# dannyfa/VAE-GAM

Hardware: AMD Instinct MI355X
Metric: fMRI volumes/sec/train-step (41x49x35) (higher is better)
Workload: dtype f32; 1 GPU; configs[2] full VAE-GAM: B=64/GPU C=8, 41x49x35, 2 subj x 98 vol synthetic checker, fwd+bwd+Adam, hipGraph replay; global_batch=64, covariates=8, parallelism=dp1

## Files before the change

vae-gam_amd/csrc/vg_conv_mm.hip:

```cpp
#include "vg_common.h"
#include <stdlib.h>
#include <stdint.h>
#include "../../include/vaegam.h"

#ifdef VG_STAMP
__device__ unsigned long long vg_stamp_out[1024 * 16 * 8];
#define VG_STAMP_T(t) do { __builtin_amdgcn_sched_barrier(0); asm volatile("s_memtime %0\n\ts_waitcnt lgkmcnt(0)" : "=s"(t) :: "memory"); __builtin_amdgcn_sched_barrier(0); } while (0)
#define VG_STAMP_ADD(i) do { unsigned long long t_; VG_STAMP_T(t_); st_sum[i] += t_ - st_last; st_last = t_; } while (0)
#else
#define VG_STAMP_ADD(i) do {} while (0)
#endif

namespace {

constexpr int MM_MAXQ = 4;
constexpr int MM_ZPAD = 64;

struct MmParams {
    vg_mm_desc d;
    int bps, nsplit;
    int ksbase[MM_MAXQ], a_off[MM_MAXQ];
    int kstot, aimg_floats;
    int a_res;
    int CHP, buf_floats;
// ... 150 lines not shown
        const char* mn = reinterpret_cast<const char*>(mask_src + (size_t)n * CO * ovol);
        const int cq = d.od0[q] * OHW + d.oh0[q] * d.OW + d.ow0[q];
#pragma unroll
        for (int i = 0; i < TPC; ++i) {
            if (i >= nact || !((vbits >> (q * TPC + i)) & 1u)) continue;
            const unsigned off = 4u * (unsigned)(ob[i] + cq);
#pragma unroll
            for (int r = 0; r < 4; ++r) {
                float v = acc[i].v[r] + bias_l[r];
                if constexpr (MASKED) {
                    if constexpr (NQ == 1) v = (mreg[i][r] > 0.f) ? v : 0.f;
                    else v = (*reinterpret_cast<const float*>(mn + (size_t)r * ovol * 4 + off) > 0.f) ? v : 0.f;
                }
#if defined(VG_ABLATE_STORE) && VG_ABLATE_STORE == 1
                if (v == 1.2345e-30f) *reinterpret_cast<float*>(yn + (size_t)r * ovol * 4 + off) = v;
#elif defined(VG_ABLATE_STORE) && VG_ABLATE_STORE == 2
                *reinterpret_cast<float*>(yn + (size_t)r * ovol * 4 + (((off >> 8) << 8) + 4u * lane)) = v;
#elif defined(VG_ABLATE_STORE) && VG_ABLATE_STORE == 4
                if (r == 0 || v == 1.2345e-30f) *reinterpret_cast<float*>(yn + (size_t)r * ovol * 4 + off) = v;
#elif defined(VG_ABLATE_STORE) && VG_ABLATE_STORE == 5
                *reinterpret_cast<float*>(yn + off) = v;
#elif defined(VG_ABLATE_STORE) && VG_ABLATE_STORE == 3
                __builtin_nontemporal_store(v, reinterpret_cast<float*>(yn + (size_t)r * ovol * 4 + off));
#else
                *reinterpret_cast<float*>(yn + (size_t)r * ovol * 4 + off) = v;
#endif
                if (stats_part) {
                    const float h = stats_relu ? vg_max(v, 0.f) : v;
                    st_s[r] += h; st_q[r] = fmaf(h, h, st_q[r]);
                }
            }
        }
    };
    auto flush_stats = [&](int n) __attribute__((always_inline)) {
        const int g = n / stats_pg;
        const size_t chunks = (size_t)stats_pg * p.bps * MM_W;
        const size_t chunkid = ((size_t)(n % stats_pg) * p.bps + b) * MM_W + wave;
#pragma unroll
        for (int r = 0; r < 4; ++r) {
            float sa = st_s[r], sb = st_q[r];
#pragma unroll
            for (int off = 8; off > 0; off >>= 1) { sa += __shfl_xor(sa, off); sb += __shfl_xor(sb, off); }
            if (CO == 8) { sa += __shfl_xor(sa, 32); sb += __shfl_xor(sb, 32); }
            if (jl == 0 && (CO == 16 || kk < 2)) {
                double* dst = stats_part + (((size_t)g * CO + co_l + r) * chunks + chunkid) * 2;
                dst[0] = (double)sa; dst[1] = (double)sb;
            }
            st_s[r] = 0.f; st_q[r] = 0.f;
        }
    };

    const int nsp = d.cc * nspan_c;
    const int parts = (nsp >= MM_W) ? 1 : (MM_W + nsp - 1) / nsp;
    const int head = dst0 & 3;
    const int n4 = (head + span_fl + 3) >> 2;
    const int n4p = (n4 + parts - 1) / parts;
    auto stage = [&](int u) __attribute__((always_inline)) {
        const int n = split + (u / nchunks) * p.nsplit, c0 = (u % nchunks) * d.cc;
        const int cc = min(d.cc, CI - c0);
        float* buf = In + (DB ? (u & 1) : 0) * p.buf_floats;
        const float* src0 = x + ((size_t)n * CI + c0) * vol + (size_t)pl_lo * IHW + (size_t)r_lo * d.IW;
        for (int it = wave; it < cc * nspan_c * parts; it += MM_W) {
            const int sp = it / parts, part = it - sp * parts;
            const int c = sp / nspan_c, pl = sp - c * nspan_c;
            const int g0 = part * n4p, g1 = min(g0 + n4p, n4);
            const int f0 = max(g0 * 4 - head, 0), f1 = min(g1 * 4 - head, span_fl);
            if (f1 > f0) vg_dma_block(src0 + (size_t)c * vol + (size_t)pl * IHW + f0, buf + c * p.CHP + MM_ZPAD + dst0 + pl * LPH + f0, f1 - f0, 0, 1, lane);
        }
    };
    auto prologue = [&](int u) __attribute__((always_inline)) {
        const int n = split + (u / nchunks) * p.nsplit, c0 = (u % nchunks) * d.cc;
        const int cc = min(d.cc, CI - c0);
        float* buf = In + (DB ? (u & 1) : 0) * p.buf_floats;
        const int g_aff = (in_scale != nullptr) ? n / d.per_group : 0;
        for (int it = wave; it < cc * nspan_c * parts; it += MM_W) {
            const int sp = it / parts, part = it - sp * parts;
            const int c = sp / nspan_c, pl = sp - c * nspan_c;
            float sc = 1.f, sh = 0.f;
            if (in_scale != nullptr) { sc = in_scale[g_aff * CI + c0 + c]; sh = in_shift[g_aff * CI + c0 + c]; }
            float* sp0 = buf + c * p.CHP + MM_ZPAD + dst0 + pl * LPH - head;
            const int g0 = part * n4p, g1 = min((part + 1) * n4p, n4);
#ifdef VG_EMU
            for (int g = g0 + lane; g < g1; g += VG_WAVE) {
                float* t = sp0 + g * 4;
#pragma unroll
                for (int e = 0; e < 4; ++e) t[e] = fmaf(vg_max(t[e], lo), sc, sh);
            }
#else
            for (int g = g0 + lane; g < g1; g += VG_WAVE) {
                const unsigned a = (unsigned)(uintptr_t)(sp0 + g * 4);
                vg_hw_f32x4 t;
                asm volatile("ds_read_b128 %0, %1\n\ts_waitcnt lgkmcnt(0)" : "=v"(t) : "v"(a) : "memory");
#pragma unroll
                for (int e = 0; e < 4; ++e) t[e] = fmaf(vg_max(t[e], lo), sc, sh);
                asm volatile("ds_write_b128 %0, %1" :: "v"(a), "v"(t) : "memory");
            }
#endif
        }
#ifndef VG_EMU
        asm volatile("s_waitcnt lgkmcnt(0)" ::: "memory");
#endif
    };
    __syncthreads();
#ifdef VG_STAMP
    unsigned long long st_sum[8] = {0, 0, 0, 0, 0, 0, 0, 0}, st_last;
    VG_STAMP_T(st_last);
#endif
    if (units > 0) stage(0);
    int g_run = -1, n_run = 0;
    int pend = 0;
    for (int u = 0; u < units; ++u) {
        const int n = split + (u / nchunks) * p.nsplit, chunk = u % nchunks, c0 = chunk * d.cc;
        const int cc = min(d.cc, CI - c0);
        float* cur = In + (DB ? (u & 1) : 0) * p.buf_floats;
        VG_STAMP_ADD(7);
        if (DB) vg_dma_wait_wave();
        else vg_wait_vm(pend);
        VG_STAMP_ADD(0);
        if (p.has_pro) prologue(u);
        VG_STAMP_ADD(1);
        __syncthreads();
        VG_STAMP_ADD(2);
        if (DB && u + 1 < units) stage(u + 1);
        if constexpr (NQ == 1 && MASKED) { if (chunk == nchunks - 1) load_mask(n); }
        VG_STAMP_ADD(3);
        auto class_work = [&](auto qc, auto ntc) __attribute__((always_inline)) {
            constexpr int q = decltype(qc)::value;
            constexpr int NT = decltype(ntc)::value;
            for (int c = 0; c < cc; ++c) {
                const float* curc = cur + c * p.CHP;
                if constexpr (STATIC_K) {
                    constexpr int KSQ = q == 0 ? K0 : q == 1 ? K1 : q == 2 ? K2 : K3;
                    constexpr int SG0 = q == 0 ? 0 : q == 1 ? K0 : q == 2 ? K0 + K1 : K0 + K1 + K2;
                    const float* Aq = Al + p.a_off[q] + (c0 + c) * KSQ * 64 + lane;
#ifdef VG_EMU
#pragma unroll
                    for (int s = 0; s < KSQ; ++s) {
                        const float aw = Aq[s * 64];
#pragma unroll
                        for (int i = 0; i < NT; ++i) vg_mfma16(aw, curc[pt[i][SG0 + s]], acc[i]);
                    }
#else
// ... 7 lines not shown
                        if (s + 1 < KSQ) {
                            asm volatile("ds_read_b32 %0, %1 offset:%2" : "=v"(a2[(s + 1) & 1]) : "v"(ab), "n"((s + 1) * 256));
#pragma unroll
                            for (int i = 0; i < NT; ++i)
                                asm volatile("ds_read_b32 %0, %1" : "=v"(b2[(s + 1) & 1][i]) : "v"(cb + 4u * (unsigned)pt[i][SG0 + s + 1]));
                            asm volatile("s_waitcnt lgkmcnt(%0)" :: "n"(NT + 1) : "memory");
                        } else {
                            asm volatile("s_waitcnt lgkmcnt(0)" ::: "memory");
                        }
                        __builtin_amdgcn_sched_barrier(0);
#pragma unroll
                        for (int i = 0; i < NT; ++i) vg_mfma16(a2[s & 1], b2[s & 1][i], acc[i]);
                        __builtin_amdgcn_sched_barrier(0);
                    }
#endif
                } else {
                    const int ksq = d.ks[q];
                    const float* Aq = Al + p.a_off[q] + (c0 + c) * ksq * 64 + lane;
                    const int* Tq = Tl + p.ksbase[q] * 64 + lane;
                    for (int s = 0; s < ksq; ++s) {
                        const float aw = Aq[s * 64];
                        const int off = Tq[s * 64] + MM_ZPAD;
                        const unsigned bit = 1u << s;
                        float bv[NT];
#pragma unroll
                        for (int i = 0; i < NT; ++i) bv[i] = curc[(vm[q][i] & bit) ? posBase[i] + off : 0];
#pragma unroll
                        for (int i = 0; i < NT; ++i) vg_mfma16(aw, bv[i], acc[i]);
                    }
                }
            }
        };
        const int g_now = stats_part ? n / stats_pg : 0;
        if (stats_part && chunk == 0 && g_run >= 0 && g_now != g_run) flush_stats(n_run);
        if constexpr (NQ == 1) {
            if (chunk == 0) zero_acc();
            if (nact > 0) mm_dispatch<TPC>(nact, [&](auto ntc) __attribute__((always_inline)) { class_work(mm_int<0>{}, ntc); });
            VG_STAMP_ADD(4);
            pend = 0;
            if constexpr (!DB) {
                if (u + 1 < units) { __syncthreads(); VG_STAMP_ADD(2); stage(u + 1); VG_STAMP_ADD(3); }
                if (chunk == nchunks - 1) pend = nst[0];
            }
            if (chunk == nchunks - 1) store_class(n, 0);
            VG_STAMP_ADD(5);
        } else {
            mm_static_for<NQ>([&](auto qc) __attribute__((always_inline)) {
                constexpr int q = decltype(qc)::value;
                zero_acc();
                VG_STAMP_ADD(5);
                if (nact > 0) mm_dispatch<TPC>(nact, [&](auto ntc) __attribute__((always_inline)) { class_work(qc, ntc); });
                VG_STAMP_ADD(4);
                if constexpr (!DB && q == NQ - 1) {
                    if (u + 1 < units) { __syncthreads(); VG_STAMP_ADD(2); stage(u + 1); VG_STAMP_ADD(3); }
                    pend = nst[q];
                }
                store_class(n, q);
            });
            VG_STAMP_ADD(5);
        }
        g_run = g_now; n_run = n;
    }
    if (stats_part && g_run >= 0) flush_stats(n_run);
    VG_STAMP_ADD(6);
#ifdef VG_STAMP
    if (lane == 0 && blockIdx.x < 1024)
        for (int i = 0; i < 8; ++i) vg_stamp_out[(blockIdx.x * 16 + wave) * 8 + i] = st_sum[i];
#endif
}

}

#ifdef VG_STAMP
extern "C" int vg_stamp_read(unsigned long long* dst, int n) {
    return (int)hipMemcpyFromSymbol(dst, HIP_SYMBOL(vg_stamp_out), sizeof(unsigned long long) * n, 0, hipMemcpyDeviceToHost);
}
#endif

static int mm_plan_params(const vg_mm_desc* d, MmParams* p, size_t* shmem, const char* who) {
    if (!d || d->N <= 0 || d->CI <= 0 || (d->CO != 8 && d->CO != 16) || d->nq < 1 || d->nq > MM_MAXQ || d->PD <= 0 || d->PDT <= 0 ||
        d->PH <= 0 || d->PW <= 0 || d->slack < 0 || d->PH > 1023 || d->PW > 1023 || d->PD > 1023 || d->cc <= 0 || d->LD <= 0 || d->tpc <= 0) {
        vg_set_error("%s: bad descriptor", who); return VG_ERR_ARG;
    }
    p->d = *d;
    int ns = 256 / p->bps; if (ns < 1) ns = 1; if (ns > d->N) ns = d->N;
    p->nsplit = ns;
    int row = 0, af = 0;
    for (int q = 0; q < d->nq; ++q) {
        if (d->ks[q] <= 0 || d->ks[q] > 32) { vg_set_error("%s: k-steps per channel must be 1..32 (class %d: %d)", who, q, d->ks[q]); return VG_ERR_ARG; }
        p->ksbase[q] = row; p->a_off[q] = af;
        row += d->ks[q]; af += d->CI * d->ks[q] * 64;
    }
    p->kstot = row; p->aimg_floats = af;
    if (d->nq > 1 && d->cc < d->CI) { vg_set_error("%s: multi-class plans need all input channels in one chunk", who); return VG_ERR_ARG; }
    const int IHW = d->IH * d->IW;
    const int W = d->waves;
// ... 92 lines not shown
```

vae-gam_amd/csrc/vg_gp.hip:

```cpp
#include "vg_common.h"
#include "../../include/vaegam.h"

namespace {

constexpr int GP_T = 256;
constexpr int GP_TB = 1024;
constexpr int GP_LDS_MAXB = 16;
constexpr int GP_NB = 16;
constexpr int GP_NBP = GP_NB + 1;
constexpr int TAB_W = 10;

struct GpLayout {
    long long Lc, A, kinv, Ls, M, N1, N2, N3, N4, T1, T2, T3, G, x, e, bm, v1, v2, v3, sc, total;
};

__host__ __device__ inline GpLayout gp_layout(long long B, long long n) {
    GpLayout w; long long o = 0;
    w.Lc = o; o += B * B;
    w.A = o; o += B * n;
    w.kinv = o; o += n * n;
    w.Ls = o; o += n * n;
    w.M = o; o += n * n;
    w.N1 = o; o += n * n; w.N2 = o; o += n * n; w.N3 = o; o += n * n; w.N4 = o; o += n * n;
    w.T1 = o; o += B * n; w.T2 = o; o += B * n; w.T3 = o; o += B * n;
// ... 231 lines not shown
            const int b = t / n, k = t % n;
            double s = 0.0;
            for (int j = 0; j < n; ++j) s += T1[b * n + j] * kinv[j * n + k];
            A[t] = s;
        }
        for (int t = tid; t < n * n; t += nt) {
            const int p = t / n, q = t % n;
            M[t] = (double)qS[t] - kvar * (kern1(fabs((double)(p - q)) * step, isl) + (p == q ? a.jitter_ku : 0.0));
        }
        __syncthreads();
        for (int b = tid; b < B; b += nt) {
            double s = 0.0;
            for (int k = 0; k < n; ++k) s += A[b * n + k] * (double)qm[k];
            if (o_fb) o_fb[(size_t)c * B + b] = s;
            bm[b] += s;
        }
        for (int t = tid; t < B * n; t += nt) {
            const int b = t / n, k = t % n;
            double s = 0.0;
            for (int j = 0; j < n; ++j) s += A[b * n + j] * M[j * n + k];
            T2[t] = s;
        }
        for (int t = tid; t < n * n; t += nt) Ls[t] = (double)qS[t];
        __syncthreads();
        chol_inplace(Ls, n);
        double part = 0.0;
        for (int t = tid; t < n * n; t += nt) {
            const int p = t / n, q = t % n;
            if (q <= p) part += Ls[t] * Ls[t] / a.prior_var;
            if (q == p) part += -2.0 * log(Ls[t]) + (double)qm[p] * (double)qm[p] / a.prior_var;
        }
        const double tot = block_sum(part, red);
        kl += 0.5 * (n * log(a.prior_var) + tot - n);
    }
    return kl;
}

template <int T>
__global__ void __launch_bounds__(T)
gain_fwd_k(GainArgs a, float* __restrict__ task_var, double* __restrict__ kl_part,
           double* __restrict__ o_bm, double* __restrict__ o_bc, double* __restrict__ o_fb, double* __restrict__ o_sg) {
    VG_DYN_SMEM(double, lds);
    double* red = lds;
    const int c = blockIdx.x, tid = threadIdx.x, nt = blockDim.x;
    const int B = a.B, n = a.n;
    const GpLayout w = gp_layout(B, n);
    double* W = a.ws + (size_t)c * w.total;
    const bool in_lds = B <= GP_LDS_MAXB;
    double* Cm = in_lds ? lds + T : W + w.Lc;
    const long long* tb = a.tab + (size_t)c * TAB_W;
    const bool is_gp = tb[0] != 0, is_hrf = tb[1] != 0;
    double* x = W + w.x; double* e = W + w.e; double* bm = W + w.bm;
    const double sa = (double)a.P[tb[3]], std_ = exp((double)a.P[tb[4]]);
    double kvar, ls, step;
    const double kl = gain_prelude(a, c, W, w, red, o_fb, kvar, ls, step);
    {
        const double* A = W + w.A; const double* T2 = W + w.T2;
        const double isl = 1.0 / sqrt(2.0) / ls;
        const double s2 = std_ * std_;
        for (long long t = tid; t < (long long)B * B; t += nt) {
            const int i = (int)(t / B), j = (int)(t % B);
            double v = (i == j) ? s2 * x[i] * x[i] : 0.0;
            if (is_gp) {
                double sg = kvar * kern1(x[j] - x[i], isl);
                for (int k = 0; k < n; ++k) sg += T2[i * n + k] * A[j * n + k];
                if (o_sg) o_sg[((size_t)c * B + i) * B + j] = sg;
                v += sg;
            }
            if (o_bc) o_bc[((size_t)c * B + i) * B + j] = v;
            Cm[t] = v + (i == j ? a.jitter_b : 0.0);
        }
        if (o_bm) for (int b = tid; b < B; b += nt) o_bm[(size_t)c * B + b] = bm[b];
    }
    __syncthreads();
    if (in_lds) chol_inplace(Cm, B);
    else chol_blocked(Cm, B, lds + T);
    if (in_lds) {
        double* Lc = W + w.Lc;
        for (long long t = tid; t < (long long)B * B; t += nt) Lc[t] = Cm[t];
    }
    double* tv = W + w.v1;
    if (in_lds) {
        for (int b = tid; b < B; b += nt) {
            double s = bm[b];
            for (int j = 0; j <= b; ++j) s += Cm[(long long)b * B + j] * e[j];
            tv[b] = s;
        }
    } else {
        const int lane = tid % VG_WAVE, wv = tid / VG_WAVE, nwv = nt / VG_WAVE;
        for (int b = wv; b < B; b += nwv) {
            double s = 0.0;
            for (int j = lane; j <= b; j += VG_WAVE) s += Cm[(long long)b * B + j] * e[j];
            for (int off = VG_WAVE / 2; off > 0; off >>= 1) s += __shfl_down(s, off);
            if (lane == 0) tv[b] = bm[b] + s;
        }
    }
    __syncthreads();
    for (int b = tid; b < B; b += nt) {
        double s = tv[b];
        if (is_hrf) {
// ... 326 lines not shown
#pragma unroll
    for (int p = 0; p < 4; ++p)
#pragma unroll
        for (int q = 0; q < 4; ++q) {
            const int i = min(i0 + ty * 4 + p, B - 1), j = min(j0 + tx * 4 + q, B - 1);
            acc[p][q] = is_gp ? kvar * kern1(x[j] - x[i], isl) : 0.0;
        }
    if (is_gp) {
        const double* A = W + w.A; const double* T2 = W + w.T2;
        double* Ts = lds; double* As = lds + GT * GTP;
        for (int k0 = 0; k0 < n; k0 += GT) {
            const int kc = min(GT, n - k0);
            __syncthreads();
            for (int t = tid; t < GT * GT; t += GP_TT) {
                const int r = t / GT, k = t % GT;
                const bool ok = k < kc;
                Ts[k * GTP + r] = (ok && i0 + r < B) ? T2[(long long)(i0 + r) * n + k0 + k] : 0.0;
                As[k * GTP + r] = (ok && j0 + r < B) ? A[(long long)(j0 + r) * n + k0 + k] : 0.0;
            }
            __syncthreads();
            mm4x4(Ts, As, kc, acc);
        }
    }
#pragma unroll
    for (int p = 0; p < 4; ++p)
#pragma unroll
        for (int q = 0; q < 4; ++q) {
            const int i = i0 + ty * 4 + p, j = j0 + tx * 4 + q;
            if (i >= B || j >= B) continue;
            double v = (i == j) ? s2 * x[i] * x[i] : 0.0;
            if (is_gp) {
                if (o_sg) o_sg[((size_t)c * B + i) * B + j] = acc[p][q];
                v += acc[p][q];
            }
            if (o_bc) o_bc[((size_t)c * B + i) * B + j] = v;
            Lc[(long long)i * B + j] = (j > i) ? 0.0 : v + (i == j ? a.jitter_b : 0.0);
        }
}

__global__ void __launch_bounds__(GP_TT)
gain_potrf_diag_k(GainArgs a, int p) {
    VG_DYN_SMEM(double, D);
    const int B = a.B, c = blockIdx.x, tid = threadIdx.x;
    const GpLayout w = gp_layout(B, a.n);
    double* Lc = a.ws + (size_t)c * w.total + w.Lc;
    const int k0 = p * GT, nb = min(GT, B - k0);
    for (int t = tid; t < nb * nb; t += GP_TT) { const int i = t / nb, j = t % nb; D[i * GTP + j] = Lc[(long long)(k0 + i) * B + k0 + j]; }
    for (int j = 0; j < nb; ++j) {
        __syncthreads();
        const double d = sqrt(D[j * GTP + j]);
        __syncthreads();
        for (int i = j + tid; i < nb; i += GP_TT) D[i * GTP + j] = (i == j) ? d : D[i * GTP + j] / d;
        __syncthreads();
        for (int t = tid; t < (nb - j - 1) * (nb - j - 1); t += GP_TT) {
            const int i = j + 1 + t / (nb - j - 1), k = j + 1 + t % (nb - j - 1);
            if (k <= i) D[i * GTP + k] -= D[i * GTP + j] * D[k * GTP + j];
        }
    }
    __syncthreads();
    for (int t = tid; t < nb * nb; t += GP_TT) { const int i = t / nb, j = t % nb; if (j <= i) Lc[(long long)(k0 + i) * B + k0 + j] = D[i * GTP + j]; }
}

__global__ void __launch_bounds__(GP_TT)
gain_potrf_panel_k(GainArgs a, int p) {
    VG_DYN_SMEM(double, lds);
    const int B = a.B, T = gt_tiles(B), tid = threadIdx.x;
// ... 453 lines not shown
```

vae-gam_amd/ops.py:

```python
import ctypes
from dataclasses import dataclass
from typing import Optional, Tuple

import torch

from . import _lib
from ._lib import ConvDesc, WgradDesc

BN_EPS = 1e-5

PROFILE = None
_LABEL = ['']


class label:
    def __init__(self, name):
        self.name = name

    def __enter__(self):
        self.prev = _LABEL[0]; _LABEL[0] = self.name

    def __exit__(self, *a):
        _LABEL[0] = self.prev

# ... 328 lines not shown
    _call(p, 'vg_bn_param_grad', _p(src), G, C, _p(dg), _p(db), 0)
    return dg, db


_GROUPED_OK = {}


def _grouped_wgrad_ok(p_shape, per_group):
    key = (tuple(p_shape), int(per_group))
    if key not in _GROUPED_OK:
        N, C, ID, IH, IW = key[0]
        d = WgradDesc(N, C, 1, ID, IH, IW, ID + 2, IH + 2, IW + 2, 3, 3, 3, 1, 0, 0, 0, 0, 0, int(per_group))
        _GROUPED_OK[key] = _lib.get_lib().dll.vg_wgrad3d_grouped_ws_bytes(ctypes.byref(d)) >= 0
    return _GROUPED_OK[key]


def bn_backward_tconv1(dy, weight, p, gamma, mean, rstd, relu, per_group, sync=None, beta=None, producer_bias_grad=None, dw_out=None):
    lib = _lib.get_lib()
    N, C = p.shape[0], p.shape[1]
    ID, IH, IW = p.shape[2:]
    assert tuple(dy.shape) == (N, 1, ID + 2, IH + 2, IW + 2) and tuple(weight.shape) == (C, 1, 3, 3, 3)
    _chk(dy); _chk(p)
    w = _chk(weight.detach().contiguous())
    G = N // per_group
    P = ID * IH * IW
    ws = torch.empty(lib.size('vg_bn_tconv1_ws_bytes', N, C, ID, per_group) // 8, dtype=torch.float64, device=p.device)
    sums = torch.empty((G * C, 2), dtype=torch.float64, device=p.device)
    if dw_out is not None:
        assert dw_out.shape == weight.shape and dw_out.is_contiguous() and dw_out.dtype == torch.float32 and beta is not None
        d = WgradDesc(N, C, 1, ID, IH, IW, ID + 2, IH + 2, IW + 2, 3, 3, 3, 1, 0, 0, 0, 0, int(relu), int(per_group))
        nbytes = lib.size('vg_wgrad3d_grouped_ws_bytes', ctypes.byref(d))
        wws = torch.empty(nbytes // 4, dtype=torch.float32, device=p.device)
        q = torch.empty((G, C + 1, 27), dtype=torch.float32, device=p.device)
        nshift = -(mean * rstd)
        _call(p, 'vg_wgrad3d_grouped', ctypes.byref(d), _p(dy), _p(p), _p(rstd), _p(nshift), _p(wws), _p(q))
        _call(p, 'vg_bn_tconv1_sums', _p(q), _p(w), _p(gamma), _p(beta), G, C, 27, _p(sums), _p(dw_out), 1)
    else:
        _call(p, 'vg_bn_bwd_reduce_tconv1', _p(dy), _p(w), _p(p), N, C, ID, IH, IW, per_group, int(relu), _p(mean), _p(rstd), _p(ws), _p(sums))
    count = float(per_group * P)
    local = None
    if sync is not None:
        local = sums.clone()
        sums = sync(sums)
        count = count * sync.world_size
    dp = torch.empty_like(p)
    if producer_bias_grad is not None:
        assert producer_bias_grad.shape == (C,) and producer_bias_grad.is_contiguous() and producer_bias_grad.dtype == torch.float32
    _call(p, 'vg_bn_bwd_apply_tconv1', _p(dy), _p(w), _p(p), _p(dp), N, C, ID, IH, IW, per_group, int(relu), _p(gamma), _p(mean), _p(rstd),
          _p(sums), count, _p(ws), _p(producer_bias_grad), 1)
    src = local if local is not None else sums
    gg, bg = _grad_buf(gamma), _grad_buf(beta)
    if gg is not None and bg is not None:
        _call(p, 'vg_bn_param_grad', _p(src), G, C, _p(gg), _p(bg), 1)
        return dp, None, None
    dg = torch.empty(C, dtype=torch.float32, device=p.device); db = torch.empty_like(dg)
    _call(p, 'vg_bn_param_grad', _p(src), G, C, _p(dg), _p(db), 0)
    return dp, dg, db


def channel_sum(x, out=None):
    lib = _lib.get_lib()
    N, C = x.shape[0], x.shape[1]
    P = x[0, 0].numel()
    ws = _bn_ws(x, N, C, P, N)
    if out is not None:
        assert out.shape == (C,) and out.is_contiguous() and out.dtype == torch.float32
        _call(x, 'vg_channel_sum', _p(_chk(x)), N, C, P, _p(ws), _p(out), 1)
# ... 2 lines not shown
    _call(x, 'vg_channel_sum', _p(_chk(x)), N, C, P, _p(ws), _p(out), 0)
    return out


class BnConvAct(torch.autograd.Function):

    @staticmethod
    def forward(ctx, p_in, weight, bias, gamma, beta, spec: ConvSpec, relu_in: bool, per_group: int,
                input_is_data: bool, sync, packed=None, next_bn=None, pre_stats=None, producer_bias=None,
                bias_grad_by_consumer=False):
        p_in = p_in.contiguous()
        has_bn = gamma is not None
        assert producer_bias is None or has_bn, 'producer_bias: the hand-off happens in the batch-norm backward'
        scale = shift = mean = rstd = None
        part = None
        with label(spec.name + '/fwd'):
            if has_bn:
                scale, shift, mean, rstd = bn_stats(p_in, gamma, beta, relu_in, per_group, sync, pre_stats)
            mmf = _mm_for(packed, weight, spec, 'fwd', tuple(p_in.shape[2:]), None)
            if mmf is not None:
                y = conv_mm(p_in, mmf[0], mmf[1], bias, relu_in, scale, shift, per_group, None, next_bn)
            else:
                wf = packed.get(spec.name, 'fwd') if packed is not None else pack_weight(weight, spec, 'fwd')
                y = conv_forward(p_in, wf, bias, spec, relu_in, scale, shift, per_group, next_bn)
            if next_bn:
                y, part = y
        ctx.spec, ctx.relu_in, ctx.per_group, ctx.input_is_data, ctx.sync, ctx.has_bn = \
            spec, relu_in, per_group, input_is_data, sync, has_bn
        ctx.save_for_backward(p_in, weight, gamma, beta, scale, shift, mean, rstd)
        ctx.bias_ref = bias
        ctx.packed = packed
        ctx.producer_bias, ctx.bias_grad_by_consumer = producer_bias, bool(bias_grad_by_consumer)
        ctx.nout = 2 if next_bn else 1
        if next_bn:
            ctx.mark_non_differentiable(part)
            return y, part
        return y

    @staticmethod
    def backward(ctx, dy, *_unused):
        with label(ctx.spec.name + '/bwd'):
            return BnConvAct._backward(ctx, dy) + (None, None, None)

    @staticmethod
    def _backward(ctx, dy):
        p_in, weight, gamma, beta, scale, shift, mean, rstd = ctx.saved_tensors
        spec, relu_in, per_group = ctx.spec, ctx.relu_in, ctx.per_group
        dy = dy.contiguous()
        wg = weight.grad if (isinstance(weight, torch.nn.Parameter) and weight.grad is not None and weight.grad.is_contiguous()) else None
        bias_t = ctx.bias_ref
        bg = bias_t.grad if (isinstance(bias_t, torch.nn.Parameter) and bias_t.grad is not None and bias_t.grad.is_contiguous()) else None
        direct_db = bg is not None and not (ctx.input_is_data and ctx.has_bn)
        overlap = direct_db and wg is not None and not ctx.input_is_data
        skip_db = ctx.bias_grad_by_consumer
        fuse_last = FUSE_LAST_BN_BWD and ctx.has_bn and not ctx.input_is_data and spec.kind == 'convt' and spec.stride == 1 \
            and spec.co == 1 and tuple(spec.k) == (3, 3, 3) and tuple(spec.pad) == (0, 0, 0) and spec.ci <= 16
        dw_by_bn = fuse_last and WGRAD_BN_SUMS and _grouped_wgrad_ok(p_in.shape, per_group)
        if dw_by_bn:
            overlap = False
        if overlap:
            with on_side_stream(dy, dy, p_in, scale, shift, wg, bg):
                if not skip_db:
                    channel_sum(dy, out=bg)
                conv_weight_grad(p_in, dy, spec, relu_in, scale, shift, per_group, out=wg)
            db = dw = None
        elif skip_db:
            db = None
        else:
            db = channel_sum(dy, out=bg) if direct_db else channel_sum(dy)
        dgamma = dbeta = dp = None
        if ctx.input_is_data:
            if ctx.has_bn:
                assert spec.kind == 'conv' and spec.pad == (0, 0, 0) and not relu_in
# ... 59 lines not shown
    if _MM_SKIP and 'k%d' % plan.ks[0] in _MM_SKIP and (plan.PDT + plan.PD - 1) // plan.PD > 1:
        return False
    if USE_MM >= 2 or (plan.PDT + plan.PD - 1) // plan.PD == 1:
        return True
    if plan.mode == 'tconv':
        return list(plan.ks) in ([3, 2, 2, 1], [2, 1, 1, 1], [2, 2, 2, 2])
    return plan.ks[0] in (7, 9)


def _mm_for(packed, weight, spec, direction, read_size, write_size):
    if not USE_MM or (direction == 'bwd' and spec.co == 1):
        return None
    if packed is not None:
        got = packed.get_mm(spec.name, direction)
        if got is not None and (got[0].ID, got[0].IH, got[0].IW) == tuple(read_size):
            return got if mm_wins(got[0]) else None
    plan = mm_plan(spec, direction, read_size, write_size)
    if not mm_wins(plan):
        return None
    return plan, plan.gather(weight)


def bn_conv_act(p_in, weight, bias, gamma, beta, spec, relu_in, per_group=None, input_is_data=False, sync=None, packed=None,
                next_bn=None, pre_stats=None, producer_bias=None, bias_grad_by_consumer=False):
    if per_group is None:
        per_group = p_in.shape[0]
    return BnConvAct.apply(p_in, weight, bias, gamma, beta, spec, relu_in, per_group, input_is_data, sync, packed, next_bn,
                           pre_stats, producer_bias, bias_grad_by_consumer)


class GamElbo(torch.autograd.Function):

    @staticmethod
    def forward(ctx, logits, gain, x, eps, glm, logits_bias=None):
        lib = _lib.get_lib()
        G, B, V = logits.shape
        C = G - 1
        logits = _chk(logits.contiguous()); gain = _chk(gain.contiguous()); x = _chk(x.contiguous())
        eps = _chk(eps.contiguous(), torch.float64); glm = _chk(glm.contiguous())
        ws = torch.empty(lib.size('vg_gam_ws_bytes', C, B, V) // 4 + 1, dtype=torch.float32, device=x.device)
        slp = torch.empty(B, dtype=torch.float32, device=x.device)
        dist = torch.empty((C, B), dtype=torch.float32, device=x.device)
        _call(x, 'vg_gam_elbo_fwd', _p(logits), _p(gain), _p(x), _p(eps), _p(glm), C, B, V, _p(ws), _p(slp), _p(dist),
                 None)
        ctx.save_for_backward(logits, gain, x, eps, glm, dist)
        ctx.logits_bias = logits_bias
        return slp, dist

    @staticmethod
    def backward(ctx, g_slp, g_dist):
        lib = _lib.get_lib()
        logits, gain, x, eps, glm, dist = ctx.saved_tensors
        tot = None
        if ctx.logits_bias is not None:
            pb = ctx.logits_bias
            assert pb.numel() == 1
            if pb.grad is None:
                raise RuntimeError('GamElbo: logits_bias.grad is not bound (see bn_conv_act: the bias gradient is added into the caller\'s buffer)')
            tot = pb.grad
        G, B, V = logits.shape
        C = G - 1
        g_slp = _chk(g_slp.contiguous()); g_dist = _chk(g_dist.contiguous())
        ws = torch.empty(lib.size('vg_gam_ws_bytes', C, B, V) // 4 + 1, dtype=torch.float32, device=x.device)
        d_logits = torch.empty_like(logits)
        d_gain = torch.empty_like(gain)
        d_eps = torch.empty_like(eps)
        _call(x, 'vg_gam_elbo_bwd', _p(logits), _p(gain), _p(x), _p(eps), _p(glm), _p(dist), _p(g_slp), _p(g_dist),
                 C, B, V, _p(ws), _p(d_logits), _p(d_gain), _p(d_eps), _p(tot), 1)
        return d_logits, d_gain, None, d_eps, None, None


class LatentSample(torch.autograd.Function):

    @staticmethod
    def forward(ctx, mu, w, a, eps_w, eps_d, G):
        B, L = mu.shape
        mu = _chk(mu.contiguous()); w = _chk(w.contiguous()); a = _chk(a.contiguous())
        eps_w = _chk(eps_w.contiguous()); eps_d = _chk(eps_d.contiguous())
        assert w.shape == (B, L) and a.shape == (B, L) and eps_d.shape == (B, L) and eps_w.numel() == B
        zcat = torch.empty((G * B, L + G), dtype=torch.float32, device=mu.device)
        kl = torch.empty(B, dtype=torch.float32, device=mu.device)
        d = torch.empty((B, L), dtype=torch.float32, device=mu.device)
        flag = torch.empty(1, dtype=torch.float32, device=mu.device)
        _call(mu, 'vg_latent_fwd', _p(mu), _p(w), _p(a), _p(eps_w), _p(eps_d), B, L, G, _p(zcat), _p(kl), _p(d), _p(flag))
        ctx.save_for_backward(mu, w, d, flag, eps_w, eps_d)
        ctx.G = G
        ctx.mark_non_differentiable(d)
        return zcat, kl, d

    @staticmethod
    def backward(ctx, g_zcat, g_kl, _g_d):
        mu, w, d, flag, eps_w, eps_d = ctx.saved_tensors
        B, L = mu.shape
        g_mu = torch.empty_like(mu); g_w = torch.empty_like(mu); g_a = torch.empty_like(mu)
        gz = _p(_chk(g_zcat.contiguous())) if g_zcat is not None else None
        gk = _p(_chk(g_kl.contiguous())) if g_kl is not None else None
        _call(mu, 'vg_latent_bwd', _p(mu), _p(w), _p(d), _p(flag), _p(eps_w), _p(eps_d), gz, gk, B, L, ctx.G,
                 _p(g_mu), _p(g_w), _p(g_a))
        return g_mu, g_w, g_a, None, None, None


class LatentSampleStacked(torch.autograd.Function):

    @staticmethod
    def forward(ctx, mwa, eps_w, eps_d, G):
        mwa = _chk(mwa.contiguous())
        _, B, L = mwa.shape
        eps_w = _chk(eps_w.contiguous()); eps_d = _chk(eps_d.contiguous())
        assert eps_d.shape == (B, L) and eps_w.numel() == B
        zcat = torch.empty((G * B, L + G), dtype=torch.float32, device=mwa.device)
        kl = torch.empty(B, dtype=torch.float32, device=mwa.device)
        d = torch.empty((B, L), dtype=torch.float32, device=mwa.device)
        flag = torch.empty(1, dtype=torch.float32, device=mwa.device)
        _call(mwa, 'vg_latent_fwd', _p(mwa[0]), _p(mwa[1]), _p(mwa[2]), _p(eps_w), _p(eps_d), B, L, G, _p(zcat), _p(kl), _p(d), _p(flag))
        ctx.save_for_backward(mwa, d, flag, eps_w, eps_d)
        ctx.G = G
        ctx.mark_non_differentiable(d)
        return zcat, kl, d

    @staticmethod
    def backward(ctx, g_zcat, g_kl, _g_d):
        mwa, d, flag, eps_w, eps_d = ctx.saved_tensors
        _, B, L = mwa.shape
        g = torch.empty_like(mwa)
        gz = _p(_chk(g_zcat.contiguous())) if g_zcat is not None else None
        gk = _p(_chk(g_kl.contiguous())) if g_kl is not None else None
        _call(mwa, 'vg_latent_bwd', _p(mwa[0]), _p(mwa[1]), _p(d), _p(flag), _p(eps_w), _p(eps_d), gz, gk, B, L, ctx.G,
                 _p(g[0]), _p(g[1]), _p(g[2]))
        return g, None, None, None


class ElboLoss(torch.autograd.Function):

    @staticmethod
    def forward(ctx, kl_z, slp, dist, gp_kl, coef):
        kl_z = _chk(kl_z.contiguous()); slp = _chk(slp.contiguous()); dist = _chk(dist.contiguous()); gp_kl = _chk(gp_kl.contiguous())
        loss = torch.empty(1, dtype=torch.float32, device=kl_z.device)
        ctx.coef = tuple(float(c) for c in coef)
        ctx.shapes = (kl_z.shape, slp.shape, dist.shape, gp_kl.shape)
        _call(kl_z, 'vg_loss_fwd', _p(kl_z), _p(slp), _p(dist), _p(gp_kl), kl_z.numel(), dist.numel(), *ctx.coef, _p(loss))
        return loss

    @staticmethod
    def backward(ctx, g):
        sk, ss, sd, sg = ctx.shapes
        g = _chk(g.contiguous())
        g_kl = torch.empty(sk, dtype=torch.float32, device=g.device); g_slp = torch.empty(ss, dtype=torch.float32, device=g.device)
        g_dist = torch.empty(sd, dtype=torch.float32, device=g.device); g_gp = torch.empty(sg, dtype=torch.float32, device=g.device)
        _call(g, 'vg_loss_bwd', _p(g), g_kl.numel(), g_dist.numel(), *ctx.coef, _p(g_kl), _p(g_slp), _p(g_dist), _p(g_gp))
        return g_kl, g_slp, g_dist, g_gp, None
# ... 172 lines not shown
        raise ValueError('%s would draw the gains of %d volumes jointly: the limit is %d volumes per joint draw (vg_gp_gain_fwd). '
                         'Use a smaller minibatch or, under data parallelism, dp_gain=\'local\' (each rank draws its own slice).'
                         % (what, int(B), GAIN_MAX_BATCH))


class GainConsts:

    def __init__(self, table, xu, hrf, n, jitter_ku=0.0, jitter_b=1e-5, prior_var=10.0):
        self.table, self.xu, self.hrf = table, xu, hrf
        self.C, self.n = int(table.shape[0]), int(n)
        self.jitter_ku, self.jitter_b, self.prior_var = float(jitter_ku), float(jitter_b), float(prior_var)

    def desc(self, B):
        return _lib.GainDesc(self.C, int(B), self.n, int(self.hrf.numel()), self.jitter_b, self.jitter_ku, self.prior_var)


class GpGain(torch.autograd.Function):

    @staticmethod
    def forward(ctx, covariates, eps_beta, consts, flat_p, flat_g, join_stream, *params):
        lib = _lib.get_lib()
        B = covariates.shape[0]
        C = consts.C
        assert covariates.dtype == torch.float32 and covariates.dim() == 2 and covariates.shape[1] >= C and covariates.stride(1) == 1
        eps_beta = _chk(eps_beta.contiguous())
        assert eps_beta.shape == (C, B)
        dev = covariates.device
        d = consts.desc(B)
        ws = torch.empty(lib.size('vg_gp_gain_ws_bytes', C, B, consts.n) // 8, dtype=torch.float64, device=dev)
        tv = torch.empty((C, B), dtype=torch.float32, device=dev)
        kl = torch.empty(1, dtype=torch.float32, device=dev)
        bm = torch.empty((C, B), dtype=torch.float64, device=dev)
        bc = torch.empty((C, B, B), dtype=torch.float64, device=dev)
        fb = torch.zeros((C, B), dtype=torch.float64, device=dev)
        sg = torch.zeros((C, B, B), dtype=torch.float64, device=dev)
        tiled = bool(GAIN_FORCE_TILED)
        _call(covariates, 'vg_gp_gain_fwd_tiled' if tiled else 'vg_gp_gain_fwd', ctypes.byref(d), _p(consts.table), _p(flat_p), _p(consts.xu), _p(covariates),
              int(covariates.stride(0)), _p(eps_beta), _p(consts.hrf), _p(ws), _p(tv), _p(kl), _p(bm), _p(bc), _p(fb), _p(sg))
        kl_terms = ws[-(C + 8):-8]
        ctx.save_for_backward(covariates, eps_beta, ws)
        ctx.consts, ctx.flat_p, ctx.flat_g, ctx.join_stream, ctx.tiled = consts, flat_p, flat_g, join_stream, tiled
        ctx.mark_non_differentiable(bm, bc, fb, sg, kl_terms)
        return tv, kl, bm, bc, fb, sg, kl_terms

    @staticmethod
    def backward(ctx, g_tv, g_kl, *_):
        covariates, eps_beta, ws = ctx.saved_tensors
        consts = ctx.consts
        B = covariates.shape[0]
        d = consts.desc(B)
        if g_tv is None:
            g_tv = torch.zeros((consts.C, B), dtype=torch.float32, device=covariates.device)
        if g_kl is None:
            g_kl = torch.zeros(1, dtype=torch.float32, device=covariates.device)
        g_tv = _chk(g_tv.contiguous()); g_kl = _chk(g_kl.contiguous())
        _call(covariates, 'vg_gp_gain_bwd_tiled' if ctx.tiled else 'vg_gp_gain_bwd', ctypes.byref(d), _p(consts.table), _p(ctx.flat_p), _p(consts.xu), _p(covariates),
              int(covariates.stride(0)), _p(eps_beta), _p(consts.hrf), _p(ws), _p(g_tv), _p(g_kl), _p(ctx.flat_g))
        if ctx.join_stream is not None and covariates.is_cuda:
            cur = torch.cuda.current_stream(covariates.device)
            if cur != ctx.join_stream:
                ctx.join_stream.wait_stream(cur)
        return (None,) * len(ctx.needs_input_grad)


class HrfAcrossRanks(torch.autograd.Function):

    @staticmethod
    def forward(ctx, pre, T, dp, lo):
        B = pre.shape[1]
        full = dp.all_gather_rows(pre.t().contiguous()).t()
        ctx.save_for_backward(T)
        ctx.dp, ctx.lo, ctx.B = dp, int(lo), int(B)
        return (full @ T)[:, lo:lo + B].contiguous()

    @staticmethod
# ... 241 lines not shown
                rows_max = min((PHB - 1) * shi + (hhi - hlo) + 1, IH)
                whole = (nslab == 1 and hlo <= 0 and (PH - 1) * shi + hhi + 1 >= IH)
                LPH = IHW if whole else ((rows_max * IW + 3) // 4) * 4 + 4
                CHP = 64 + ((LD * LPH + 63) // 64) * 64
                bps = ((PDT + PD - 1) // PD) * nslab
                for cc in ([CI] if nq > 1 else [c for c in range(CI, 0, -1) if CI % c == 0]):
                    for dbuf in (1, 0):
                        if pin and (W, PD, PHB, cc, dbuf) != tuple(pin):
                            continue
                        lds = (((aidx.size + 63) // 64) * 64 + rows * 64 + (1 + dbuf) * cc * CHP + 64) * 4
                        if lds > _MM_LDS_BUDGET:
                            continue
                        per_simd = 4 if (tpc <= 3 or nq > 1) else 2
                        nblk = min(_MM_LDS_CU // lds, per_simd * 4 // W)
                        if nblk < 1:
                            continue
                        util = npos / float(tpc * W * 16) * (PDT / float(((PDT + PD - 1) // PD) * PD)) * (PH / float(nslab * PHB))
                        halo = ((PD * sdi) / float(LD)) * min(1.0, (PHB * shi) / float(rows_max))
                        wps = nblk * W // 4
                        occ = {1: 0.45, 2: 0.6, 3: 0.8}.get(wps, 1.0)
                        shape = (1.0 if nslab == 1 else 0.85) * (1.0 if W == 8 else 0.9)
                        score = util * (0.5 + 0.5 * halo) * (0.9 + 0.1 * cc / float(CI)) * occ * shape * (1.0 if (dbuf or nblk >= 2) else 0.9)
                        cands.append((score, PD, LD, cc, tpc, dbuf, PHB, W))
    if not cands:
        return None
    _, PD, LD, cc, tpc, dbuf, PHB, W = max(cands, key=lambda c: (round(c[0], 9), c[3], -c[5]))
    tpc = {1: (3 if tpc <= 3 else tpc if tpc <= 6 else 8), 4: 4}[nq]
    return MmPlan(CI=CI, CO=CO, ID=ID, IH=IH, IW=IW, OD=OD, OH=OH, OW=OW, nq=nq, ks=ks, PDT=PDT, PH=PH, PW=PW, PD=PD, sdi=sdi, shi=shi,
                  swi=swi, d0=d0, LD=LD, cc=cc, sdo=sdo, sho=sho, swo=swo, od0=od0, oh0=oh0, ow0=ow0, tpc=tpc, slack=slack, dbuf=dbuf,
                  PHB=PHB, hlo=hlo, hhi=hhi, waves=W,
                  tau=tau.reshape(-1), dlt=dlt.reshape(-1), aidx=aidx, mode=mode)


def conv_mm(x, plan: MmPlan, aimg, bias, relu_in, scale, shift, per_group, mask_src=None, next_bn=None):
    lib = _lib.get_lib()
    N = x.shape[0]
    assert tuple(x.shape[1:]) == (plan.CI, plan.ID, plan.IH, plan.IW), (tuple(x.shape), plan.CI, plan.ID, plan.IH, plan.IW)
    tau, dlt, _ = plan.tables(x.device)
    d = plan.desc(N, relu_in, per_group if scale is not None else 1)
    y = torch.empty((N, plan.CO, plan.OD, plan.OH, plan.OW), dtype=torch.float32, device=x.device)
    _chk(x); _chk(aimg)
    if next_bn:
        chunks = lib.size('vg_conv_mm_stats_chunks', ctypes.byref(d), int(next_bn))
        G = N // int(next_bn)
        part = torch.zeros(G * plan.CO * chunks * 2, dtype=torch.float64, device=x.device)
        _call(x, 'vg_conv_mm', ctypes.byref(d), _p(x), _p(aimg), _p(tau), _p(dlt), _p(bias), _p(scale), _p(shift), _p(mask_src), _p(y),
              int(next_bn), 1, _p(part))
        return y, part
    _call(x, 'vg_conv_mm', ctypes.byref(d), _p(x), _p(aimg), _p(tau), _p(dlt), _p(bias), _p(scale), _p(shift), _p(mask_src), _p(y), 1, 0, None)
    return y
```

vae-gam_amd/vae_reg_GP.py:

```python
import datetime
import os

import numpy as np
import torch
import torch.utils.data
from torch import nn
from torch.nn import functional as F

from . import gp, ops, utils
from .optim import FusedAdam
from .schema import REF_CSV_COLS, REF_IMG_KEYS, covariate_schema, net_geometry, parameter_sets

IMG_SHAPE = (41, 49, 35)
IMG_DIM = int(np.prod(IMG_SHAPE))


class _NullWriter:
    def __getattr__(self, name):
        return lambda *a, **k: None


class _JsonlWriter(_NullWriter):
    def __init__(self, log_dir):
        import json
# ... 378 lines not shown
        eps_beta = noise['eps_beta'] if (joint_gains or W == 1) else noise['eps_beta'][:, lo:lo + B].contiguous()
        hrf_rows = [i for i, c in enumerate(self.schema) if c.hrf]
        hrf_across = W > 1 and not joint_gains and bool(hrf_rows)
        gains_stream = self._gains_stream(dev)
        if gains_stream is not None:
            main = torch.cuda.current_stream(dev)
            gains_stream.wait_stream(main)
        heads = self._encode_heads(x, stacked=True)
        if gains_stream is not None:
            with torch.cuda.stream(gains_stream):
                gains = self._gains(covariates, eps_beta, join_stream=main, hrf_in_kernel=not hrf_across)
        else:
            gains = self._gains(covariates, eps_beta, hrf_in_kernel=not hrf_across)
        G = C + 1
        if torch.is_tensor(heads):
            zcat, kl_z, d = ops.LatentSampleStacked.apply(heads, eps_w, eps_d, G)
            mu, w = heads[0], heads[1]
        else:
            mu, w, a = heads
            zcat, kl_z, d = ops.LatentSample.apply(mu, w, a, eps_w, eps_d, G)
        z, u = zcat[:B, :L], w.unsqueeze(-1)
        logits = self._decode_logits(zcat, B, last_bias_by_consumer=True).view(G, B, self.img_dim)
        task_var, gp_kl_loss, beta_mean, beta_cov, post = gains
        if gains_stream is not None:
            torch.cuda.current_stream(dev).wait_stream(gains_stream)
            for t in (task_var, gp_kl_loss):
                t.record_stream(torch.cuda.current_stream(dev))
        if joint_gains:
            task_var = task_var[:, lo:lo + B].contiguous()
        if hrf_across:
            conv = ops.HrfAcrossRanks.apply(task_var[hrf_rows], self._hrf_matrix(Bg, dev), self.dp, lo)
            task_var = torch.cat([conv[hrf_rows.index(i)].unsqueeze(0) if i in hrf_rows else task_var[i:i + 1] for i in range(C)], 0)
        xf = x.reshape(B, self.img_dim)
        slp, dist = ops.GamElbo.apply(logits, task_var, xf, self.epsilon.view(-1), self._glm(), self.convt5.bias)
        loss = ops.ElboLoss.apply(kl_z, slp, dist, gp_kl_loss,
                                  (1.0 / Bg, -1.0 / Bg, self._gp_kl_scale_host / W, float(self.glm_reg_scale) * Bg))
        out = dict(loss=loss, z=z, mu=mu, u=u, d=d, kl_z=kl_z, task_var=task_var, gp_kl_loss=gp_kl_loss,
                   sum_log_prob=slp, dist=dist, logits=logits, beta_mean=beta_mean, beta_cov=beta_cov,
                   gp_post=post)
        if want_maps:
            out['maps'] = ops.gam_maps(logits.detach(), task_var.detach(), xf, self.epsilon.detach().view(-1), self._glm())
        return out

    def forward(self, ids, covariates, x, log_type, return_latent_rec=False, train_mode=True, noise=None):
        want_maps = return_latent_rec or (train_mode and self.log_maps)
        out = self.forward_core(covariates, x, noise, want_maps)
        if train_mode and self.log_maps:
            maps = out['maps']
            for sl in (12, 15, 18):
                utils.log_map(self.writer, self.img_shape, maps[0], sl, 'base_map', ids.shape[0], log_type)
                utils.log_map(self.writer, self.img_shape, maps[1], sl, 'task_map', ids.shape[0], log_type)
                utils.log_map(self.writer, self.img_shape, maps[-1], sl, 'full_reconstruction', ids.shape[0], log_type)
        if return_latent_rec:
            maps = out['maps'].cpu().numpy()
            imgs = {k: {} for k in REF_IMG_KEYS} if self.num_covariates <= 8 else {}
            imgs['base'] = maps[0]
            for i, c in enumerate(self.schema, start=1):
                imgs[c.img_key] = maps[i]
            imgs['full_rec'] = maps[-1]
            return out['loss'], out['z'].detach().cpu().numpy(), imgs
        return out['loss']

    def _batch_to_device(self, sample):
        x = sample['volume'].to(self.device, non_blocking=True)
        covariates = sample['covariates'].to(self.device, non_blocking=True)
        ids = sample['subjid'].to(self.device, non_blocking=True)
        return ids, covariates, x

    def train_step(self, ids, covariates, x, noise=None):
        self.check_gain_batch(x.shape[0])
        if self.use_hip_graph and noise is None and x.is_cuda:
            g = self._graphs.get(tuple(x.shape))
            if g is None:
                g = self._capture_step(ids, covariates, x)
            if g is not False:
                g['x'].copy_(x, non_blocking=True); g['cov'].copy_(covariates, non_blocking=True)
                Bg = x.shape[0] * (1 if self.dp is None else self.dp.world_size)
                self.draw_noise(Bg, x.device, out=g['noise'])
                g['graph'].replay()
                self.optimizer.step_count += 1
                return g['loss']
        return self._train_step_eager(ids, covariates, x, noise)

    def _train_step_eager(self, ids, covariates, x, noise=None):
        self.optimizer.zero_grad()
        loss = self.forward(ids, covariates, x, 'train', train_mode=True, noise=noise)
        loss.backward()
        ops.join_side_stream(x.device)
        if self.dp is not None:
            self.dp.allreduce_grads(self.optimizer.flat_grads())
        self.optimizer.advance()
        self.optimizer.apply_update()
        loss = loss.detach()
        if self.dp is not None:
            loss = self.dp.sum_scalar_tensor(loss)
        return loss

    def _capture_step(self, ids, covariates, x):
        import warnings
        key = tuple(x.shape)
        st = {'x': x.clone(), 'cov': covariates.clone(), 'ids': ids.clone()}
        snap = [(g, g['p'].clone(), g['m'].clone(), g['v'].clone()) for g in self.optimizer.groups.values()]
        counters = self.optimizer.counters_snapshot()
        torch.cuda.current_stream(x.device).synchronize()
        rng = torch.cuda.get_rng_state(x.device)
        try:
            if self.dp is not None and self.dp._host_staging:
                raise RuntimeError('collectives staged through the host (gloo) cannot be captured')
            st['noise'] = self.draw_noise(x.shape[0] * (1 if self.dp is None else self.dp.world_size), x.device)
            side = torch.cuda.Stream()
            side.wait_stream(torch.cuda.current_stream())
            with torch.cuda.stream(side):
                for _ in range(2):
                    self._train_step_eager(st['ids'], st['cov'], st['x'], noise=st['noise'])
            torch.cuda.current_stream().wait_stream(side)
            graph = torch.cuda.CUDAGraph()
            with torch.cuda.graph(graph):
                try:
                    st['loss'] = self._train_step_eager(st['ids'], st['cov'], st['x'], noise=st['noise'])
                except Exception:
# ... 272 lines not shown
```

Before: 9956 volumes/s.

## Drop redundant zero-fills, memsets and grad materialization in train step

```diff
diff --git a/vae-gam_amd/csrc/vg_conv_mm.hip b/vae-gam_amd/csrc/vg_conv_mm.hip
--- a/vae-gam_amd/csrc/vg_conv_mm.hip
+++ b/vae-gam_amd/csrc/vg_conv_mm.hip
@@ -206,7 +206,7 @@
             }
         }
     };
-    auto flush_stats = [&](int n) __attribute__((always_inline)) {
+    auto flush_stats = [&](int n0, int n) __attribute__((always_inline)) {
         const int g = n / stats_pg;
         const size_t chunks = (size_t)stats_pg * p.bps * MM_W;
         const size_t chunkid = ((size_t)(n % stats_pg) * p.bps + b) * MM_W + wave;
@@ -217,7 +217,12 @@
             for (int off = 8; off > 0; off >>= 1) { sa += __shfl_xor(sa, off); sb += __shfl_xor(sb, off); }
             if (CO == 8) { sa += __shfl_xor(sa, 32); sb += __shfl_xor(sb, 32); }
             if (jl == 0 && (CO == 16 || kk < 2)) {
-                double* dst = stats_part + (((size_t)g * CO + co_l + r) * chunks + chunkid) * 2;
+                double* row = stats_part + ((size_t)g * CO + co_l + r) * chunks * 2;
+                for (int m = n0; m < n; m += p.nsplit) {
+                    double* z = row + (((size_t)(m % stats_pg) * p.bps + b) * MM_W + wave) * 2;
+                    z[0] = 0.0; z[1] = 0.0;
+                }
+                double* dst = row + chunkid * 2;
                 dst[0] = (double)sa; dst[1] = (double)sb;
             }
             st_s[r] = 0.f; st_q[r] = 0.f;
@@ -281,7 +286,7 @@
     VG_STAMP_T(st_last);
 #endif
     if (units > 0) stage(0);
-    int g_run = -1, n_run = 0;
+    int g_run = -1, n_run = 0, n_run0 = 0;
     int pend = 0;
     for (int u = 0; u < units; ++u) {
         const int n = split + (u / nchunks) * p.nsplit, chunk = u % nchunks, c0 = chunk * d.cc;
@@ -355,7 +360,8 @@
             }
         };
         const int g_now = stats_part ? n / stats_pg : 0;
-        if (stats_part && chunk == 0 && g_run >= 0 && g_now != g_run) flush_stats(n_run);
+        if (stats_part && chunk == 0 && g_run >= 0 && g_now != g_run) flush_stats(n_run0, n_run);
+        if (g_now != g_run) n_run0 = n;
         if constexpr (NQ == 1) {
             if (chunk == 0) zero_acc();
             if (nact > 0) mm_dispatch<TPC>(nact, [&](auto ntc) __attribute__((always_inline)) { class_work(mm_int<0>{}, ntc); });
@@ -384,7 +390,7 @@
         }
         g_run = g_now; n_run = n;
     }
-    if (stats_part && g_run >= 0) flush_stats(n_run);
+    if (stats_part && g_run >= 0) flush_stats(n_run0, n_run);
     VG_STAMP_ADD(6);
 #ifdef VG_STAMP
     if (lane == 0 && blockIdx.x < 1024)
diff --git a/vae-gam_amd/csrc/vg_gp.hip b/vae-gam_amd/csrc/vg_gp.hip
--- a/vae-gam_amd/csrc/vg_gp.hip
+++ b/vae-gam_amd/csrc/vg_gp.hip
@@ -287,6 +287,8 @@
         }
         const double tot = block_sum(part, red);
         kl += 0.5 * (n * log(a.prior_var) + tot - n);
+    } else if (o_fb) {
+        for (int b = tid; b < B; b += nt) o_fb[(size_t)c * B + b] = 0.0;
     }
     return kl;
 }
@@ -321,6 +323,8 @@
                 for (int k = 0; k < n; ++k) sg += T2[i * n + k] * A[j * n + k];
                 if (o_sg) o_sg[((size_t)c * B + i) * B + j] = sg;
                 v += sg;
+            } else if (o_sg) {
+                o_sg[((size_t)c * B + i) * B + j] = 0.0;
             }
             if (o_bc) o_bc[((size_t)c * B + i) * B + j] = v;
             Cm[t] = v + (i == j ? a.jitter_b : 0.0);
@@ -713,6 +717,8 @@
             if (is_gp) {
                 if (o_sg) o_sg[((size_t)c * B + i) * B + j] = acc[p][q];
                 v += acc[p][q];
+            } else if (o_sg) {
+                o_sg[((size_t)c * B + i) * B + j] = 0.0;
             }
             if (o_bc) o_bc[((size_t)c * B + i) * B + j] = v;
             Lc[(long long)i * B + j] = (j > i) ? 0.0 : v + (i == j ? a.jitter_b : 0.0);
diff --git a/vae-gam_amd/ops.py b/vae-gam_amd/ops.py
--- a/vae-gam_amd/ops.py
+++ b/vae-gam_amd/ops.py
@@ -384,7 +384,8 @@
         nbytes = lib.size('vg_wgrad3d_grouped_ws_bytes', ctypes.byref(d))
         wws = torch.empty(nbytes // 4, dtype=torch.float32, device=p.device)
         q = torch.empty((G, C + 1, 27), dtype=torch.float32, device=p.device)
-        nshift = -(mean * rstd)
+        nshift = torch.empty_like(mean)
+        _call(mean, 'vg_data_bn_nshift', _p(_chk(mean)), _p(_chk(rstd)), mean.numel(), _p(nshift))
         _call(p, 'vg_wgrad3d_grouped', ctypes.byref(d), _p(dy), _p(p), _p(rstd), _p(nshift), _p(wws), _p(q))
         _call(p, 'vg_bn_tconv1_sums', _p(q), _p(w), _p(gamma), _p(beta), G, C, 27, _p(sums), _p(dw_out), 1)
     else:
@@ -453,6 +454,7 @@
         ctx.packed = packed
         ctx.producer_bias, ctx.bias_grad_by_consumer = producer_bias, bool(bias_grad_by_consumer)
         ctx.nout = 2 if next_bn else 1
+        ctx.set_materialize_grads(False)
         if next_bn:
             ctx.mark_non_differentiable(part)
             return y, part
@@ -460,6 +462,8 @@
 
     @staticmethod
     def backward(ctx, dy, *_unused):
+        if dy is None:
+            return (None,) * 15
         with label(ctx.spec.name + '/bwd'):
             return BnConvAct._backward(ctx, dy) + (None, None, None)
 
@@ -585,7 +589,7 @@
 class GamElbo(torch.autograd.Function):
 
     @staticmethod
-    def forward(ctx, logits, gain, x, eps, glm, logits_bias=None):
+    def forward(ctx, logits, gain, x, eps, glm, logits_bias=None, eps_param=None):
         lib = _lib.get_lib()
         G, B, V = logits.shape
         C = G - 1
@@ -598,6 +602,7 @@
                  None)
         ctx.save_for_backward(logits, gain, x, eps, glm, dist)
         ctx.logits_bias = logits_bias
+        ctx.eps_param = eps_param
         return slp, dist
 
     @staticmethod
@@ -617,10 +622,13 @@
         ws = torch.empty(lib.size('vg_gam_ws_bytes', C, B, V) // 4 + 1, dtype=torch.float32, device=x.device)
         d_logits = torch.empty_like(logits)
         d_gain = torch.empty_like(gain)
-        d_eps = torch.empty_like(eps)
+        ep = ctx.eps_param
+        eps_direct = ep is not None and ep.grad is not None and ep.grad.is_contiguous() and ep.grad.dtype == eps.dtype \
+            and ep.grad.numel() == eps.numel()
+        d_eps = ep.grad.view(eps.shape) if eps_direct else torch.empty_like(eps)
         _call(x, 'vg_gam_elbo_bwd', _p(logits), _p(gain), _p(x), _p(eps), _p(glm), _p(dist), _p(g_slp), _p(g_dist),
                  C, B, V, _p(ws), _p(d_logits), _p(d_gain), _p(d_eps), _p(tot), 1)
-        return d_logits, d_gain, None, d_eps, None, None
+        return d_logits, d_gain, None, (None if eps_direct else d_eps), None, None, None
 
 
 class LatentSample(torch.autograd.Function):
@@ -639,6 +647,7 @@
         ctx.save_for_backward(mu, w, d, flag, eps_w, eps_d)
         ctx.G = G
         ctx.mark_non_differentiable(d)
+        ctx.set_materialize_grads(False)
         return zcat, kl, d
 
     @staticmethod
@@ -669,6 +678,7 @@
         ctx.save_for_backward(mwa, d, flag, eps_w, eps_d)
         ctx.G = G
         ctx.mark_non_differentiable(d)
+        ctx.set_materialize_grads(False)
         return zcat, kl, d
 
     @staticmethod
@@ -907,8 +917,8 @@
         kl = torch.empty(1, dtype=torch.float32, device=dev)
         bm = torch.empty((C, B), dtype=torch.float64, device=dev)
         bc = torch.empty((C, B, B), dtype=torch.float64, device=dev)
-        fb = torch.zeros((C, B), dtype=torch.float64, device=dev)
-        sg = torch.zeros((C, B, B), dtype=torch.float64, device=dev)
+        fb = torch.empty((C, B), dtype=torch.float64, device=dev)
+        sg = torch.empty((C, B, B), dtype=torch.float64, device=dev)
         tiled = bool(GAIN_FORCE_TILED)
         _call(covariates, 'vg_gp_gain_fwd_tiled' if tiled else 'vg_gp_gain_fwd', ctypes.byref(d), _p(consts.table), _p(flat_p), _p(consts.xu), _p(covariates),
               int(covariates.stride(0)), _p(eps_beta), _p(consts.hrf), _p(ws), _p(tv), _p(kl), _p(bm), _p(bc), _p(fb), _p(sg))
@@ -916,6 +926,7 @@
         ctx.save_for_backward(covariates, eps_beta, ws)
         ctx.consts, ctx.flat_p, ctx.flat_g, ctx.join_stream, ctx.tiled = consts, flat_p, flat_g, join_stream, tiled
         ctx.mark_non_differentiable(bm, bc, fb, sg, kl_terms)
+        ctx.set_materialize_grads(False)
         return tv, kl, bm, bc, fb, sg, kl_terms
 
     @staticmethod
@@ -1223,7 +1234,7 @@
                   tau=tau.reshape(-1), dlt=dlt.reshape(-1), aidx=aidx, mode=mode)
 
 
-def conv_mm(x, plan: MmPlan, aimg, bias, relu_in, scale, shift, per_group, mask_src=None, next_bn=None):
+def conv_mm(x, plan: MmPlan, aimg, bias, relu_in, scale, shift, per_group, mask_src=None, next_bn=None, part=None):
     lib = _lib.get_lib()
     N = x.shape[0]
     assert tuple(x.shape[1:]) == (plan.CI, plan.ID, plan.IH, plan.IW), (tuple(x.shape), plan.CI, plan.ID, plan.IH, plan.IW)
@@ -1234,7 +1245,9 @@
     if next_bn:
         chunks = lib.size('vg_conv_mm_stats_chunks', ctypes.byref(d), int(next_bn))
         G = N // int(next_bn)
-        part = torch.zeros(G * plan.CO * chunks * 2, dtype=torch.float64, device=x.device)
+        if part is None:
+            part = torch.empty(G * plan.CO * chunks * 2, dtype=torch.float64, device=x.device)
+        assert part.dtype == torch.float64 and part.is_contiguous() and part.numel() == G * plan.CO * chunks * 2
         _call(x, 'vg_conv_mm', ctypes.byref(d), _p(x), _p(aimg), _p(tau), _p(dlt), _p(bias), _p(scale), _p(shift), _p(mask_src), _p(y),
               int(next_bn), 1, _p(part))
         return y, part
diff --git a/vae-gam_amd/vae_reg_GP.py b/vae-gam_amd/vae_reg_GP.py
--- a/vae-gam_amd/vae_reg_GP.py
+++ b/vae-gam_amd/vae_reg_GP.py
@@ -434,7 +434,7 @@
             conv = ops.HrfAcrossRanks.apply(task_var[hrf_rows], self._hrf_matrix(Bg, dev), self.dp, lo)
             task_var = torch.cat([conv[hrf_rows.index(i)].unsqueeze(0) if i in hrf_rows else task_var[i:i + 1] for i in range(C)], 0)
         xf = x.reshape(B, self.img_dim)
-        slp, dist = ops.GamElbo.apply(logits, task_var, xf, self.epsilon.view(-1), self._glm(), self.convt5.bias)
+        slp, dist = ops.GamElbo.apply(logits, task_var, xf, self.epsilon.view(-1), self._glm(), self.convt5.bias, self.epsilon)
         loss = ops.ElboLoss.apply(kl_z, slp, dist, gp_kl_loss,
                                   (1.0 / Bg, -1.0 / Bg, self._gp_kl_scale_host / W, float(self.glm_reg_scale) * Bg))
         out = dict(loss=loss, z=z, mu=mu, u=u, d=d, kl_z=kl_z, task_var=task_var, gp_kl_loss=gp_kl_loss,
@@ -487,7 +487,10 @@
     def _train_step_eager(self, ids, covariates, x, noise=None):
         self.optimizer.zero_grad()
         loss = self.forward(ids, covariates, x, 'train', train_mode=True, noise=noise)
-        loss.backward()
+        one = getattr(self, '_loss_seed', None)
+        if one is None or one.device != loss.device or one.shape != loss.shape or one.dtype != loss.dtype:
+            one = self._loss_seed = torch.ones_like(loss)
+        loss.backward(one)
         ops.join_side_stream(x.device)
         if self.dp is not None:
             self.dp.allreduce_grads(self.optimizer.flat_grads())
```

Measured after the change: 9967 volumes/s, median of 4. No clear change (+0.1%).
